# microsoft/GenerativeImage2Text

Hardware: AMD Instinct MI355X
Metric: captions/sec whole-node (GIT_BASE 224px bs=64/GPU greedy len=20) (higher is better)
Workload: dtype f16; 1 GPU; GIT_BASE 224px bs=64/GPU greedy max_len=20 frames=1; global_batch=64, parallelism=dp1, decode_steps_per_caption=19, seq_len_returned=20, hip_graph=True, contexts_in_flight=4, layernorm_folded=True, library=libgitmi_f16.so, encoder_chains=2, schedule=mixed

## Files before the change

generativeimage2text_amd/csrc/kernels_gemm10.hip:

```cpp
#include "gitmi_common.h"
#include "launchers.h"
#include <type_traits>

namespace gitmi {

namespace {

constexpr int BN = 256, BK = 64;
constexpr int HALF_BYTES = 128 * BK * 2;
constexpr int BUF_BYTES = 4 * HALF_BYTES;
constexpr int LDS_BYTES = 2 * BUF_BYTES;
constexpr int SLOT_A0 = 0, SLOT_A1 = HALF_BYTES, SLOT_B0 = 2 * HALF_BYTES, SLOT_B1 = 3 * HALF_BYTES;

typedef __attribute__((address_space(3))) void lds_void_t;

#define P8_BARRIER()                           \
    do {                                       \
        __builtin_amdgcn_sched_barrier(0);     \
        __builtin_amdgcn_s_barrier();          \
        asm volatile("" ::: "memory");         \
        __builtin_amdgcn_sched_barrier(0);     \
    } while (0)

__device__ __forceinline__ float add_unfused(float a, float b) {
#pragma clang fp contract(off)
    return a + b;
}

__device__ __forceinline__ void half_wave_sum2_hi(float& a, float& b) {
    asm volatile(
        "s_nop 1\n\t"
        "v_add_f32_dpp %0, %0, %0 quad_perm:[1,0,3,2] row_mask:0xf bank_mask:0xf\n\t"
        "v_add_f32_dpp %1, %1, %1 quad_perm:[1,0,3,2] row_mask:0xf bank_mask:0xf\n\t"
        "s_nop 0\n\t"
        "v_add_f32_dpp %0, %0, %0 quad_perm:[2,3,0,1] row_mask:0xf bank_mask:0xf\n\t"
        "v_add_f32_dpp %1, %1, %1 quad_perm:[2,3,0,1] row_mask:0xf bank_mask:0xf\n\t"
        "s_nop 0\n\t"
        "v_add_f32_dpp %0, %0, %0 row_ror:4 row_mask:0xf bank_mask:0xf\n\t"
        "v_add_f32_dpp %1, %1, %1 row_ror:4 row_mask:0xf bank_mask:0xf\n\t"
        "s_nop 0\n\t"
        "v_add_f32_dpp %0, %0, %0 row_ror:8 row_mask:0xf bank_mask:0xf\n\t"
        "v_add_f32_dpp %1, %1, %1 row_ror:8 row_mask:0xf bank_mask:0xf\n\t"
        "s_nop 0\n\t"
        "v_add_f32_dpp %0, %0, %0 row_bcast:15 row_mask:0xa bank_mask:0xf\n\t"
        "v_add_f32_dpp %1, %1, %1 row_bcast:15 row_mask:0xa bank_mask:0xf\n\t"
        "s_nop 1"
        : "+v"(a), "+v"(b));
}

#define P8_LDS_BARRIER()                                   \
    do {                                                   \
        asm volatile("s_waitcnt lgkmcnt(0)" ::: "memory"); \
        __builtin_amdgcn_s_barrier();                      \
        asm volatile("" ::: "memory");                     \
    } while (0)

template <typename T> __device__ __forceinline__ uint32_t pack2o(float lo, float hi) {
    if constexpr (std::is_same<T, f16_t>::value) return pack2h(lo, hi);
    else return pack2bf(lo, hi);
}
template <typename T> __device__ __forceinline__ void unpack2o(uint32_t u, float& lo, float& hi) {
    if constexpr (std::is_same<T, f16_t>::value) unpack2h(u, lo, hi);
    else unpack2op(u, lo, hi);
}

template <int N> __device__ __forceinline__ void wait_vm() {
    if constexpr (N == 8) asm volatile("s_waitcnt vmcnt(8)" ::: "memory");
    else if constexpr (N == 4) asm volatile("s_waitcnt vmcnt(4)" ::: "memory");
    else if constexpr (N == 2) asm volatile("s_waitcnt vmcnt(2)" ::: "memory");
    else if constexpr (N == 0) asm volatile("s_waitcnt vmcnt(0)" ::: "memory");
}

template <typename TOut, int ACT, int DBG = 0, int MH = 128, int EPI = 1, int MH1 = MH, int LNF = 0>
__global__ __launch_bounds__(512) void gemm_p8_kernel(GemmArgs g) {
    static_assert(LNF == 0 || sizeof(TOut) == 2, "LayerNorm folding: 16-bit outputs only");
    static_assert(MH % 32 == 0 && MH1 % 32 == 0 && MH1 <= MH && MH <= 128, "half tiles: multiples of 32 rows, second <= first");
    constexpr int BM = MH + MH1, MI = MH / 32, MI1 = MH1 / 32;
    __shared__ __attribute__((aligned(16))) unsigned char smem[LDS_BYTES];

    const int tid = threadIdx.x;
    const int lane = tid & 63;
    const int wave = __builtin_amdgcn_readfirstlane(tid >> 6);
    const int grp = wave >> 2, wc = wave & 3;
    const int l15 = lane & 15, lg = lane >> 4;
    uint64_t ts[8];
    auto stamp = [&](int i) {
        if constexpr ((DBG & 16) != 0) {
            __builtin_amdgcn_sched_barrier(0);
            ts[2 * i] = __builtin_amdgcn_s_memtime();
            ts[2 * i + 1] = __builtin_amdgcn_s_memrealtime();
            __builtin_amdgcn_sched_barrier(0);
        }
    };
    auto stamps_out = [&]() {
        if constexpr ((DBG & 16) != 0) {
            if (tid == 0) {
                uint64_t* o = reinterpret_cast<uint64_t*>(const_cast<float*>(g.res)) + (size_t)blockIdx.x * 8;
#pragma unroll
                for (int i = 0; i < 8; ++i) o[i] = ts[i];
            }
        }
    };
    stamp(0);

    int tile_m, tile_n;
    {
        const int x = blockIdx.x & 7, idx = blockIdx.x >> 3;
        const int ng = g.ng, mg = 8 / ng;
        const int gn = x % ng, gm = x / ng;
        const int tiles_m = (g.M + BM - 1) / BM;
        const int n_lo = gn * g.tiles_n / ng, n_hi = (gn + 1) * g.tiles_n / ng;
        const int nn = n_hi - n_lo;
        const int tg = tiles_m * nn;
        const int lo_t = gm * tg / mg, hi_t = (gm + 1) * tg / mg;
        if (idx >= hi_t - lo_t) return;
        const int L = lo_t + idx;
        tile_m = L / nn;
        tile_n = n_lo + L % nn;
    }
    const int m0 = tile_m * BM, n0 = tile_n * BN;

    const char* __restrict__ Ab = reinterpret_cast<const char*>(g.A);
    const char* __restrict__ Wb = reinterpret_cast<const char*>(g.W);

    const int Rl = lane >> 4, hi = (lane >> 3) & 1, lo = lane & 7;
    uint32_t a_off[2][2], w_off[2][2];
#pragma unroll
    for (int h = 0; h < 2; ++h)
#pragma unroll
        for (int q = 0; q < 2; ++q) {
            const int rr = h * MH + (wave * 2 + q) * 8 + 2 * Rl + (hi ^ q);
            const int ch = lo ^ (q * 4 + Rl);
            int m = m0 + rr;
            m = m < g.M ? m : g.M - 1;
            a_off[h][q] = ((uint32_t)m * (uint32_t)g.lda + ch * 8) * 2u;
            const int rn = h * 128 + (wave * 2 + q) * 8 + 2 * Rl + (hi ^ q);
            w_off[h][q] = ((uint32_t)(n0 + rn) * (uint32_t)g.K + ch * 8) * 2u;
        }
    auto issue = [&](int isw, int half, int kt) {
        if constexpr (DBG & 8) return;
        const char* src = (isw ? Wb : Ab) + (size_t)kt * (BK * 2);
        unsigned char* dst = smem + (kt & 1) * BUF_BYTES + (isw ? SLOT_B0 : SLOT_A0) + half * HALF_BYTES + wave * 2048;
        const uint32_t o0 = isw ? w_off[half][0] : a_off[half][0];
        const uint32_t o1 = isw ? w_off[half][1] : a_off[half][1];
        __builtin_amdgcn_global_load_lds((const void*)(src + o0), (lds_void_t*)(dst), 16, 0, 0);
        __builtin_amdgcn_global_load_lds((const void*)(src + o1), (lds_void_t*)(dst + 1024), 16, 0, 0);
    };

    const int rowpart = (l15 >> 1) * 256 + ((l15 & 1) ^ ((l15 >> 3) & 1)) * 128;
    const int x7 = (l15 >> 1) & 7;
    const int ch0 = ((0 * 4 + lg) ^ x7) * 16;
    const int ch1 = ((1 * 4 + lg) ^ x7) * 16;
    const int a_rd = grp * (MH / 2) * 128 + rowpart;
    const int a_rd1 = grp * (MH1 / 2) * 128 + rowpart + HALF_BYTES;
    const int w_rd = SLOT_B0 + wc * 32 * 128 + rowpart;

    f32x4_t acc[2][2][2][MI];

    bf16x8_t af[MI][2], wf0[2][2], wf1[2][2];

    auto read_a = [&](const unsigned char* sb, auto half_c) {
        if constexpr (DBG & 4) return;
        constexpr int half = decltype(half_c)::value;
        const int base = half ? a_rd1 : a_rd;
#pragma unroll
        for (int i = 0; i < (half ? MI1 : MI); ++i) {
            af[i][0] = *reinterpret_cast<const bf16x8_t*>(sb + base + i * 2048 + ch0);
            af[i][1] = *reinterpret_cast<const bf16x8_t*>(sb + base + i * 2048 + ch1);
        }
    };
    constexpr std::integral_constant<int, 0> H0{};
    constexpr std::integral_constant<int, 1> H1{};
    auto read_w = [&](const unsigned char* sb, int half, bf16x8_t (&wf)[2][2]) {
        if constexpr (DBG & 4) return;
#pragma unroll
        for (int j = 0; j < 2; ++j) {
            wf[j][0] = *reinterpret_cast<const bf16x8_t*>(sb + w_rd + half * HALF_BYTES + j * 2048 + ch0);
            wf[j][1] = *reinterpret_cast<const bf16x8_t*>(sb + w_rd + half * HALF_BYTES + j * 2048 + ch1);
        }
    };
    auto mma = [&](f32x4_t (&c)[2][MI], const bf16x8_t (&wf)[2][2], auto half_c) {
        if constexpr (DBG & 4) return;
        constexpr int MIq = decltype(half_c)::value ? MI1 : MI;
        __builtin_amdgcn_s_setprio(1);
#pragma unroll
        for (int kk = 0; kk < 2; ++kk)
#pragma unroll
            for (int j = 0; j < 2; ++j)
#pragma unroll
                for (int i = 0; i < MIq; ++i)
                    c[j][i] = mfma16(wf[j][kk], af[i][kk], c[j][i]);
        __builtin_amdgcn_s_setprio(0);
    };

    auto ktile = [&](auto mode_c, int t) {
        constexpr int MODE = decltype(mode_c)::value;
        const unsigned char* sb = smem + (t & 1) * BUF_BYTES;
        read_w(sb, 0, wf0);
        __builtin_amdgcn_sched_barrier(0);
        read_a(sb, H0);
        if constexpr (MODE <= 1) { issue(1, 1, t + 1); wait_vm<8>(); } else { wait_vm<2>(); }
        P8_BARRIER();
        mma(acc[0][0], wf0, H0);
        P8_BARRIER();
        read_w(sb, 1, wf1);
        if constexpr (MODE <= 1) { issue(0, 1, t + 1); wait_vm<8>(); } else { wait_vm<0>(); }
        P8_BARRIER();
        mma(acc[0][1], wf1, H0);
        P8_BARRIER();
        read_a(sb, H1);
        if constexpr (MODE == 0) { issue(0, 0, t + 2); wait_vm<8>(); }
        P8_BARRIER();
        mma(acc[1][1], wf1, H1);
        P8_BARRIER();
        if constexpr (MODE == 0) { issue(1, 0, t + 2); wait_vm<8>(); }
        else if constexpr (MODE == 1) { wait_vm<4>(); }
        P8_BARRIER();
        mma(acc[1][0], wf0, H1);
        P8_BARRIER();
    };

    float lmean[2][MI], lrstd[2][MI];
    unsigned char* const ln_lds = smem + BUF_BYTES + SLOT_A1;
    if constexpr (LNF == 1) {
        const int r = lane >> 1, qm = r >> 4, l = r & 15;
        const int MHq = qm ? MH1 : MH, MIq = qm ? MI1 : MI;
        const int ii = wc < MIq ? wc : MIq - 1;
        const int m = m0 + qm * MH + grp * (MHq / 2) + ii * 16 + l;
        const int mc = m < g.M ? m : g.M - 1;
        const char* src = reinterpret_cast<const char*>(g.ln_part) + (size_t)mc * 32 + (lane & 1) * 16;
        __builtin_amdgcn_global_load_lds((const void*)src, (lds_void_t*)(ln_lds + wave * 1024), 16, 0, 0);
    }
    auto ln_rows = [&]() {
        if constexpr (LNF == 1) {
#pragma unroll
            for (int qm = 0; qm < 2; ++qm) {
                const int MIq = qm ? MI1 : MI;
                const int ii = lg < MIq ? lg : MIq - 1;
                const unsigned char* pr = ln_lds + (grp * 4 + ii) * 1024 + (qm * 16 + l15) * 32;
                const f32x4_t p0 = *reinterpret_cast<const f32x4_t*>(pr);
                const f32x4_t p1 = *reinterpret_cast<const f32x4_t*>(pr + 16);
                const float sx = (p0[0] + p0[2]) + (p1[0] + p1[2]);
                const float sq = (p0[1] + p0[3]) + (p1[1] + p1[3]);
                const float mean = sx * g.ln_inv_d;
                const float rstd = rsqrtf(fmaxf(sq * g.ln_inv_d - mean * mean, 0.f) + g.ln_eps);
#pragma unroll
                for (int i = 0; i < MIq; ++i) {
                    lmean[qm][i] = __shfl(mean, i * 16 + l15, 64);
                    lrstd[qm][i] = __shfl(rstd, i * 16 + l15, 64);
                    asm volatile("" : "+v"(lmean[qm][i]), "+v"(lrstd[qm][i]));
                }
            }
            __builtin_amdgcn_sched_barrier(0);
        }
    };
    const int nk = g.K / BK;
    issue(0, 0, 0); issue(1, 0, 0); issue(1, 1, 0); issue(0, 1, 0); issue(0, 0, 1); issue(1, 0, 1);
    wait_vm<8>();
    P8_BARRIER();
    ln_rows();
#pragma unroll
    for (int a = 0; a < 2; ++a)
#pragma unroll
        for (int b = 0; b < 2; ++b)
#pragma unroll
            for (int j = 0; j < 2; ++j)
#pragma unroll
                for (int i = 0; i < MI; ++i) acc[a][b][j][i] = f32x4_t{0.f, 0.f, 0.f, 0.f};
    if (grp == 1) P8_BARRIER();
    stamp(1);
    for (int t = 0; t < nk - 2; ++t) ktile(std::integral_constant<int, 0>{}, t);
    ktile(std::integral_constant<int, 1>{}, nk - 2);
    ktile(std::integral_constant<int, 2>{}, nk - 1);
    if (grp == 0) P8_BARRIER();
    stamp(2);

    constexpr int NQN = sizeof(TOut) == 2 ? 2 : 1;
    constexpr int WCOL = 128 * NQN;
    constexpr int EPC = 16 / (int)sizeof(TOut);
    constexpr int EPS = WCOL + EPC;
    constexpr int CPR = WCOL / EPC;
    static_assert(MH * EPS * sizeof(TOut) <= LDS_BYTES && (MH * CPR) % 512 == 0 && (MH1 * CPR) % 512 == 0, "epilogue slab does not fit");
    TOut* ep = reinterpret_cast<TOut*>(smem);
    TOut* __restrict__ C = reinterpret_cast<TOut*>(g.C);

    if constexpr (DBG & 2) {
        float sum = 0.f;
#pragma unroll
        for (int a = 0; a < 2; ++a)
#pragma unroll
            for (int b = 0; b < 2; ++b)
#pragma unroll
                for (int j = 0; j < 2; ++j)
#pragma unroll
                    for (int i = 0; i < MI; ++i) sum += acc[a][b][j][i][0] + acc[a][b][j][i][1] + acc[a][b][j][i][2] + acc[a][b][j][i][3];
        if (sum == 12345.678f) C[0] = (TOut)0;
        stamp(3);
        stamps_out();
        return;
    }
    f32x4_t bias4[2][2];
#pragma unroll
    for (int qn = 0; qn < 2; ++qn)
#pragma unroll
        for (int j = 0; j < 2; ++j)
            bias4[qn][j] = g.bias ? *reinterpret_cast<const f32x4_t*>(g.bias + n0 + qn * 128 + wc * 32 + j * 16 + lg * 4)
                                  : f32x4_t{0.f, 0.f, 0.f, 0.f};

    f32x4_t cs4[2][2];
    if constexpr (LNF == 1) {
#pragma unroll
        for (int qn = 0; qn < 2; ++qn)
#pragma unroll
            for (int j = 0; j < 2; ++j)
                cs4[qn][j] = *reinterpret_cast<const f32x4_t*>(g.ln_colsum + n0 + qn * 128 + wc * 32 + j * 16 + lg * 4);
    }
    auto ln_apply = [&](float a, int qm, int qn, int j, int i, int r) -> float {
        if constexpr (LNF == 1) return lrstd[qm][i] * fmaf(-lmean[qm][i], cs4[qn][j][r], a);
        else return a;
    };

    if constexpr (sizeof(TOut) == 4 && EPI == 1) {
        float* Cf = reinterpret_cast<float*>(g.C);
        const float* R = g.res;
        const int col0 = n0 + wc * 32 + lg * 4;
        const bool has_res = R != nullptr && !(DBG & 1);
#pragma unroll
        for (int qm = 0; qm < 2; ++qm) {
            const int MIq = qm ? MI1 : MI, MHq = qm ? MH1 : MH;
            f32x4_t rr[MI][2][2];
            if (has_res) {
#pragma unroll
                for (int i = 0; i < MIq; ++i) {
                    const int m = m0 + qm * MH + grp * (MHq / 2) + i * 16 + l15;
                    const int mc = m < g.M ? m : g.M - 1;
                    const float* rp = R + (size_t)mc * g.ldr + col0;
#pragma unroll
                    for (int qn = 0; qn < 2; ++qn)
#pragma unroll
                        for (int j = 0; j < 2; ++j)
                            rr[i][qn][j] = *reinterpret_cast<const f32x4_t*>(rp + qn * 128 + j * 16);
                }
            }
#pragma unroll
            for (int i = 0; i < MIq; ++i) {
                const int m = m0 + qm * MH + grp * (MHq / 2) + i * 16 + l15;
                float* cp = Cf + (size_t)m * g.ldc + col0;
                const bool ok = m < g.M && !(DBG & 1);
#pragma unroll
                for (int qn = 0; qn < 2; ++qn)
#pragma unroll
                    for (int j = 0; j < 2; ++j) {
                        f32x4_t v;
#pragma unroll
                        for (int r = 0; r < 4; ++r) v[r] = apply_act_t<ACT>(acc[qm][qn][j][i][r] + bias4[qn][j][r]);
                        if (has_res) {
#pragma unroll
                            for (int r = 0; r < 4; ++r) v[r] = add_unfused(v[r], rr[i][qn][j][r]);
                        }
                        if (ok) *reinterpret_cast<f32x4_t*>(cp + qn * 128 + j * 16) = v;
                    }
            }
        }
        return;
    }

    float rgm[8], rbt[8];
    if constexpr (LNF == 2) {
        if (g.res_part) {
            ld8(g.res_gamma + n0 + (tid & 31) * 8, rgm);
            ld8(g.res_beta + n0 + (tid & 31) * 8, rbt);
        }
    }
#pragma unroll
    for (int qm = 0; qm < 2; ++qm)
#pragma unroll
        for (int s = 0; s < 2 / NQN; ++s) {
            const int MIq = qm ? MI1 : MI, MHq = qm ? MH1 : MH;
#pragma unroll
            for (int u = 0; u < NQN; ++u) {
                const int qn = s * NQN + u;
#pragma unroll
                for (int j = 0; j < 2; ++j) {
                    const int nl = u * 128 + wc * 32 + j * 16 + lg * 4;
#pragma unroll
                    for (int i = 0; i < MIq; ++i) {
                        float v[4];
#pragma unroll
                        for (int r = 0; r < 4; ++r) v[r] = apply_act_t<ACT>(ln_apply(acc[qm][qn][j][i][r], qm, qn, j, i, r) + bias4[qn][j][r]);
                        TOut* p = ep + (grp * (MHq / 2) + i * 16 + l15) * EPS + nl;
                        if constexpr (sizeof(TOut) == 4) {
                            *reinterpret_cast<f32x4_t*>(p) = f32x4_t{v[0], v[1], v[2], v[3]};
                        } else {
                            uint2 t2;
                            t2.x = pack2o<TOut>(v[0], v[1]);
                            t2.y = pack2o<TOut>(v[2], v[3]);
                            *reinterpret_cast<uint2*>(p) = t2;
                        }
                    }
                }
            }
            P8_LDS_BARRIER();
#pragma unroll 4
            for (int q = 0; q < MHq * CPR / 512; ++q) {
                const int chunk = tid + q * 512;
                const int row = chunk / CPR, cc = chunk % CPR;
                const int m = m0 + qm * MH + row;
                const int n = n0 + s * WCOL + cc * EPC;
                if (m < g.M && !(DBG & 1)) {
                    if constexpr (sizeof(TOut) == 4) {
                        f32x4_t v = *reinterpret_cast<const f32x4_t*>(ep + row * EPS + cc * EPC);
                        if (g.res && !(DBG & 16)) {
                            const f32x4_t rr = *reinterpret_cast<const f32x4_t*>(g.res + (size_t)m * g.ldr + n);
                            v[0] += rr[0]; v[1] += rr[1]; v[2] += rr[2]; v[3] += rr[3];
                        }
                        *reinterpret_cast<f32x4_t*>(C + (size_t)m * g.ldc + n) = v;
                    } else if constexpr (LNF == 2) {
                    } else {
                        u32x4_t v = *reinterpret_cast<const u32x4_t*>(ep + row * EPS + cc * EPC);
                        if (g.res && !(DBG & 16)) {
                            float f[8], rs[8];
#pragma unroll
                            for (int e = 0; e < 4; ++e) unpack2o<TOut>(v[e], f[2 * e], f[2 * e + 1]);
                            if constexpr (std::is_same<TOut, f16_t>::value) {
                                const u32x4_t rr = *reinterpret_cast<const u32x4_t*>(reinterpret_cast<const f16_t*>(g.res) + (size_t)m * g.ldr + n);
#pragma unroll
                                for (int e = 0; e < 4; ++e) unpack2h(rr[e], rs[2 * e], rs[2 * e + 1]);
                            } else {
                                const float* rp = g.res + (size_t)m * g.ldr + n;
                                const f32x4_t r0 = *reinterpret_cast<const f32x4_t*>(rp);
                                const f32x4_t r1 = *reinterpret_cast<const f32x4_t*>(rp + 4);
#pragma unroll
                                for (int e = 0; e < 4; ++e) { rs[e] = r0[e]; rs[4 + e] = r1[e]; }
                            }
#pragma unroll
                            for (int e = 0; e < 8; ++e) f[e] += rs[e];
#pragma unroll
                            for (int e = 0; e < 4; ++e) v[e] = pack2o<TOut>(f[2 * e], f[2 * e + 1]);
                        }
                        TOut* cp = C + (size_t)m * g.ldc + n;
                        if (g.dbg & 512)
                            *reinterpret_cast<u32x4_t*>(cp) = v;
                        else
                            asm volatile("global_store_dwordx4 %0, %1, off sc1\n\ts_nop 1" ::"v"(cp), "v"(v) : "memory");
                    }
                }
                if constexpr (LNF == 2) {
                    static_assert(LNF != 2 || CPR == 32, "one stream row per half wave");
                    const bool ok = m < g.M;
                    const int mc = ok ? m : g.M - 1;
                    u32x4_t v = *reinterpret_cast<const u32x4_t*>(ep + row * EPS + cc * EPC);
                    float f[8];
#pragma unroll
                    for (int e = 0; e < 4; ++e) unpack2h(v[e], f[2 * e], f[2 * e + 1]);
                    if (g.res) {
                        float rs[8];
                        const u32x4_t rr = *reinterpret_cast<const u32x4_t*>(reinterpret_cast<const f16_t*>(g.res) + (size_t)mc * g.ldr + n);
#pragma unroll
                        for (int e = 0; e < 4; ++e) unpack2h(rr[e], rs[2 * e], rs[2 * e + 1]);
                        if (g.res_part) {
                            const f32x4_t* pp = reinterpret_cast<const f32x4_t*>(g.res_part + (size_t)mc * 4);
                            const f32x4_t p0 = pp[0], p1 = pp[1];
                            const float mean = ((p0[0] + p0[2]) + (p1[0] + p1[2])) * g.res_inv_d;
                            const float rstd = rsqrtf(fmaxf(((p0[1] + p0[3]) + (p1[1] + p1[3])) * g.res_inv_d - mean * mean, 0.f) + g.res_eps);
#pragma unroll
                            for (int e = 0; e < 8; ++e) rs[e] = fmaf((rs[e] - mean) * rstd, rgm[e], rbt[e]);
                        }
#pragma unroll
                        for (int e = 0; e < 8; ++e) f[e] += rs[e];
#pragma unroll
                        for (int e = 0; e < 4; ++e) v[e] = pack2h(f[2 * e], f[2 * e + 1]);
                    }
                    if (g.part_out) {
                        typedef __attribute__((ext_vector_type(2))) float f32x2_t;
                        f32x2_t s2 = {0.f, 0.f}, q2 = {0.f, 0.f};
#pragma unroll
                        for (int e = 0; e < 4; ++e) {
                            float x0, x1;
                            unpack2h(v[e], x0, x1);
                            const f32x2_t x = {x0, x1};
                            s2 += x;
                            q2 = __builtin_elementwise_fma(x, x, q2);
                        }
                        float sx = s2[0] + s2[1], sq = q2[0] + q2[1];
                        half_wave_sum2_hi(sx, sq);
                        if (ok && cc == 16 && !(DBG & 1)) g.part_out[(size_t)m * 4 + tile_n] = float2{sx, sq};
                    }
                    if (ok && !(DBG & 1)) {
                        TOut* cp = C + (size_t)m * g.ldc + n;
                        asm volatile("global_store_dwordx4 %0, %1, off sc1\n\ts_nop 1" ::"v"(cp), "v"(v) : "memory");
                    }
                }
            }
            P8_LDS_BARRIER();
        }
    if constexpr ((DBG & 16) != 0) {
        asm volatile("s_waitcnt vmcnt(0)" ::: "memory");
        stamp(3);
        stamps_out();
    }
}

}

template <typename TOut, int MH, int EPI = 1, int MH1 = MH, int LNF = 0>
static void launch_p8_t(const GemmArgs& g, hipStream_t s) {
    if constexpr (LNF == 2) {
        hipLaunchKernelGGL((gemm_p8_kernel<TOut, GITMI_ACT_NONE, 0, MH, EPI, MH1, LNF>), dim3(g.nwg), dim3(512), 0, s, g);
        return;
    } else {
    if (g.dbg && LNF == 0) {
        if constexpr (MH == 128 && MH1 == 128) {
            switch (g.dbg) {
                case 1: hipLaunchKernelGGL((gemm_p8_kernel<TOut, 0, 1>), dim3(g.nwg), dim3(512), 0, s, g); return;
                case 2: hipLaunchKernelGGL((gemm_p8_kernel<TOut, 0, 2>), dim3(g.nwg), dim3(512), 0, s, g); return;
                case 6: hipLaunchKernelGGL((gemm_p8_kernel<TOut, 0, 6>), dim3(g.nwg), dim3(512), 0, s, g); return;
                case 10: hipLaunchKernelGGL((gemm_p8_kernel<TOut, 0, 10>), dim3(g.nwg), dim3(512), 0, s, g); return;
#ifdef GITMI_PROBE
                case 16: hipLaunchKernelGGL((gemm_p8_kernel<TOut, 0, 16>), dim3(g.nwg), dim3(512), 0, s, g); return;
                case 17: hipLaunchKernelGGL((gemm_p8_kernel<TOut, 0, 17>), dim3(g.nwg), dim3(512), 0, s, g); return;
                case 18: hipLaunchKernelGGL((gemm_p8_kernel<TOut, 0, 18>), dim3(g.nwg), dim3(512), 0, s, g); return;
                case 22: hipLaunchKernelGGL((gemm_p8_kernel<TOut, 0, 22>), dim3(g.nwg), dim3(512), 0, s, g); return;
                case 26: hipLaunchKernelGGL((gemm_p8_kernel<TOut, 0, 26>), dim3(g.nwg), dim3(512), 0, s, g); return;
#endif
                default: break;
            }
        }
    }
    switch (g.act) {
        case GITMI_ACT_QUICKGELU:
            hipLaunchKernelGGL((gemm_p8_kernel<TOut, GITMI_ACT_QUICKGELU, 0, MH, EPI, MH1, LNF>), dim3(g.nwg), dim3(512), 0, s, g); break;
        case GITMI_ACT_GELU_ERF:
            hipLaunchKernelGGL((gemm_p8_kernel<TOut, GITMI_ACT_GELU_ERF, 0, MH, EPI, MH1, LNF>), dim3(g.nwg), dim3(512), 0, s, g); break;
        default:
            hipLaunchKernelGGL((gemm_p8_kernel<TOut, GITMI_ACT_NONE, 0, MH, EPI, MH1, LNF>), dim3(g.nwg), dim3(512), 0, s, g); break;
    }
    }
}

bool gemm_p8_supports(const GemmArgs& g) {
    return g.K % BK == 0 && g.K >= 2 * BK && g.N % BN == 0 &&
           (double)g.M * g.lda * 2.0 < 4.0e9 && (double)g.N * g.K * 2.0 < 4.0e9;
}

static int p8_xcd_count(const GemmArgs& g, int bm, int ng, int* max_nn_out) {
    const int tiles_m = (g.M + bm - 1) / bm, tiles_n = g.N / BN, mg = 8 / ng;
    int max_cnt = 0, max_nn = 0;
    for (int x = 0; x < 8; ++x) {
        const int gn = x % ng, gm = x / ng;
        const int nn = (gn + 1) * tiles_n / ng - gn * tiles_n / ng;
        const int tg = tiles_m * nn;
        const int cnt = (gm + 1) * tg / mg - gm * tg / mg;
        max_cnt = cnt > max_cnt ? cnt : max_cnt;
        max_nn = nn > max_nn ? nn : max_nn;
    }
    if (max_nn_out) *max_nn_out = max_nn;
    return max_cnt;
}
static int p8_plan(const GemmArgs& g, int bm, int* ng_out, int* max_cnt_out) {
    const int tiles_n = g.N / BN;
    int best_ng = 1, best_rounds = 1 << 30, best_cnt = 0, best_panels = 1 << 30;
    for (int ng = 1; ng <= 8 && ng <= tiles_n; ng *= 2) {
        int max_nn = 0;
        const int max_cnt = p8_xcd_count(g, bm, ng, &max_nn);
        const int rounds = (max_cnt + 31) / 32;
        const int panels = (32 + max_nn - 1) / max_nn + (max_nn < 32 ? max_nn : 32);
        if (rounds < best_rounds || (rounds == best_rounds && panels < best_panels)) {
            best_ng = ng; best_rounds = rounds; best_cnt = max_cnt; best_panels = panels;
        }
    }
    if (ng_out) *ng_out = best_ng;
    if (max_cnt_out) *max_cnt_out = best_cnt;
    return best_rounds;
}

int gemm_p8_cost(const GemmArgs& g, int bm) {
    const int rounds = p8_plan(g, bm, nullptr, nullptr);
    const int ktile = 1450 * (90 + 166 * bm / 256) / 256;
    return rounds * (1450 + (g.K / BK) * ktile + 4700 * bm / 256);
}

template <int MH, int MH1>
static void launch_p8_height(const GemmArgs& g, bool out_f32, bool staged, hipStream_t s) {
#ifdef GITMI_OPS_F16
    if (g.ln_part) { launch_p8_t<bf16_t, MH, 1, MH1, 1>(g, s); return; }
    if (g.part_out || g.res_part) { launch_p8_t<f16_t, MH, 1, MH1, 2>(g, s); return; }
#endif
    if (g.out_f16) launch_p8_t<f16_t, MH, 1, MH1>(g, s);
    else if (!out_f32) launch_p8_t<bf16_t, MH, 1, MH1>(g, s);
    else if (staged) launch_p8_t<float, MH, 0, MH1>(g, s);
    else launch_p8_t<float, MH, 1, MH1>(g, s);
}

hipError_t launch_gemm_p8(GemmArgs g, bool out_f32, hipStream_t s) {
    if (g.ln_part || g.part_out || g.res_part) {
#ifndef GITMI_OPS_F16
        return hipErrorInvalidValue;
#endif
        if (g.ln_part && (out_f32 || g.out_f16 || g.res || !g.ln_colsum || g.ln_nparts < 1 || g.part_out || g.res_part)) return hipErrorInvalidValue;
        if ((g.part_out || g.res_part) && (!g.out_f16 || out_f32 || g.act != 0 || g.N > 1024)) return hipErrorInvalidValue;
        if (g.res_part && (!g.res || !g.res_gamma || !g.res_beta || g.res_nparts < 1)) return hipErrorInvalidValue;
    }
    static const int heights[5] = {256, 224, 192, 160, 128};
    int bm = 256;
    if (!g.shared) {
        int best = gemm_p8_cost(g, 256);
        for (int h = 1; h < 5; ++h) {
            const int c = gemm_p8_cost(g, heights[h]);
            if (c < best) { best = c; bm = heights[h]; }
        }
    }
    if (g.dbg & 64) bm = 192;
    if (g.dbg & 128) bm = 256;
    if (g.dbg & 16384) bm = 160;
    if (g.dbg & 32768) bm = 224;
    if (g.dbg & 65536) bm = 128;
    g.dbg &= ~(64 | 128 | 16384 | 32768 | 65536);
    g.tiles_n = g.N / BN;
    int max_cnt = 0;
    p8_plan(g, bm, &g.ng, &max_cnt);
    if (g.dbg & (1024 | 2048 | 4096 | 8192)) {
        const int ng = (g.dbg & 1024) ? 1 : (g.dbg & 2048) ? 2 : (g.dbg & 4096) ? 4 : 8;
        g.dbg &= ~(1024 | 2048 | 4096 | 8192);
        if (ng <= g.tiles_n) { g.ng = ng; max_cnt = p8_xcd_count(g, bm, ng, nullptr); }
    }
    g.nwg = 8 * max_cnt;
    const bool staged = (g.dbg & 256) != 0;
    g.dbg &= ~256;
    switch (bm) {
        case 224: launch_p8_height<128, 96>(g, out_f32, staged, s); break;
        case 192: launch_p8_height<96, 96>(g, out_f32, staged, s); break;
        case 160: launch_p8_height<96, 64>(g, out_f32, staged, s); break;
        case 128: launch_p8_height<64, 64>(g, out_f32, staged, s); break;
        default: launch_p8_height<128, 128>(g, out_f32, staged, s); break;
    }
    return hipGetLastError();
}

}
```

Baseline: 11510 captions/s.

## Park LayerNorm row stats in LDS and pack epilogue math into float2

Per-row LayerNorm mean and rstd are no longer held in registers through the main loop. They are written to an extra LDS region and reloaded only in the epilogue, which is meant to cut VGPR pressure during the MMA loop. The bias, LN fold and activation math is rewritten on float2 vectors so it can use packed FP32 instructions. Store addressing is hoisted into a per-thread slab pointer, and the residual add is skipped for LNF paths. This adds LDS usage and a dependence on the layout of the parked stats.

```diff
diff --git a/generativeimage2text_amd/csrc/kernels_gemm10.hip b/generativeimage2text_amd/csrc/kernels_gemm10.hip
--- a/generativeimage2text_amd/csrc/kernels_gemm10.hip
+++ b/generativeimage2text_amd/csrc/kernels_gemm10.hip
@@ -64,6 +64,34 @@
     else unpack2op(u, lo, hi);
 }
 
+typedef __attribute__((ext_vector_type(2))) float f32x2_t;
+template <int ACT> __device__ __forceinline__ f32x2_t apply_act2(f32x2_t x) {
+    if constexpr (ACT == GITMI_ACT_QUICKGELU) {
+        const f32x2_t a = (x * -1.702f) * 1.4426950408889634f;
+        const f32x2_t d = f32x2_t{__builtin_amdgcn_exp2f(a[0]), __builtin_amdgcn_exp2f(a[1])} + 1.0f;
+        return x * f32x2_t{fast_rcp(d[0]), fast_rcp(d[1])};
+    } else if constexpr (ACT == GITMI_ACT_GELU_ERF) {
+        const f32x2_t one = {1.0f, 1.0f};
+        const f32x2_t z = x * 0.70710678118654752440f;
+        const f32x2_t az = __builtin_elementwise_abs(z);
+        const f32x2_t d = __builtin_elementwise_fma(f32x2_t{0.3275911f, 0.3275911f}, az, one);
+        const f32x2_t t = {fast_rcp(d[0]), fast_rcp(d[1])};
+        f32x2_t poly = {1.061405429f, 1.061405429f};
+        poly = __builtin_elementwise_fma(poly, t, f32x2_t{-1.453152027f, -1.453152027f});
+        poly = __builtin_elementwise_fma(poly, t, f32x2_t{1.421413741f, 1.421413741f});
+        poly = __builtin_elementwise_fma(poly, t, f32x2_t{-0.284496736f, -0.284496736f});
+        poly = __builtin_elementwise_fma(poly, t, f32x2_t{0.254829592f, 0.254829592f});
+        poly = poly * t;
+        const f32x2_t a = (-az * az) * 1.4426950408889634f;
+        const f32x2_t ex = {__builtin_amdgcn_exp2f(a[0]), __builtin_amdgcn_exp2f(a[1])};
+        const f32x2_t e = __builtin_elementwise_fma(-poly, ex, one);
+        const f32x2_t se = {copysignf(e[0], z[0]), copysignf(e[1], z[1])};
+        return (x * 0.5f) * (se + 1.0f);
+    } else {
+        return x;
+    }
+}
+
 template <int N> __device__ __forceinline__ void wait_vm() {
     if constexpr (N == 8) asm volatile("s_waitcnt vmcnt(8)" ::: "memory");
     else if constexpr (N == 4) asm volatile("s_waitcnt vmcnt(4)" ::: "memory");
@@ -76,7 +104,8 @@
     static_assert(LNF == 0 || sizeof(TOut) == 2, "LayerNorm folding: 16-bit outputs only");
     static_assert(MH % 32 == 0 && MH1 % 32 == 0 && MH1 <= MH && MH <= 128, "half tiles: multiples of 32 rows, second <= first");
     constexpr int BM = MH + MH1, MI = MH / 32, MI1 = MH1 / 32;
-    __shared__ __attribute__((aligned(16))) unsigned char smem[LDS_BYTES];
+    constexpr int PARK_BYTES = LNF == 1 ? 8 * 2 * 16 * 4 * (int)sizeof(float2) : 0;
+    __shared__ __attribute__((aligned(16))) unsigned char smem[LDS_BYTES + PARK_BYTES];
 
     const int tid = threadIdx.x;
     const int lane = tid & 63;
@@ -220,7 +249,7 @@
         P8_BARRIER();
     };
 
-    float lmean[2][MI], lrstd[2][MI];
+    float2* const ln_park = reinterpret_cast<float2*>(smem + LDS_BYTES);
     unsigned char* const ln_lds = smem + BUF_BYTES + SLOT_A1;
     if constexpr (LNF == 1) {
         const int r = lane >> 1, qm = r >> 4, l = r & 15;
@@ -244,12 +273,7 @@
                 const float sq = (p0[1] + p0[3]) + (p1[1] + p1[3]);
                 const float mean = sx * g.ln_inv_d;
                 const float rstd = rsqrtf(fmaxf(sq * g.ln_inv_d - mean * mean, 0.f) + g.ln_eps);
-#pragma unroll
-                for (int i = 0; i < MIq; ++i) {
-                    lmean[qm][i] = __shfl(mean, i * 16 + l15, 64);
-                    lrstd[qm][i] = __shfl(rstd, i * 16 + l15, 64);
-                    asm volatile("" : "+v"(lmean[qm][i]), "+v"(lrstd[qm][i]));
-                }
+                ln_park[((wave * 2 + qm) * 16 + l15) * 4 + lg] = float2{mean, rstd};
             }
             __builtin_amdgcn_sched_barrier(0);
         }
@@ -315,10 +339,6 @@
             for (int j = 0; j < 2; ++j)
                 cs4[qn][j] = *reinterpret_cast<const f32x4_t*>(g.ln_colsum + n0 + qn * 128 + wc * 32 + j * 16 + lg * 4);
     }
-    auto ln_apply = [&](float a, int qm, int qn, int j, int i, int r) -> float {
-        if constexpr (LNF == 1) return lrstd[qm][i] * fmaf(-lmean[qm][i], cs4[qn][j][r], a);
-        else return a;
-    };
 
     if constexpr (sizeof(TOut) == 4 && EPI == 1) {
         float* Cf = reinterpret_cast<float*>(g.C);
@@ -377,6 +397,16 @@
 #pragma unroll
         for (int s = 0; s < 2 / NQN; ++s) {
             const int MIq = qm ? MI1 : MI, MHq = qm ? MH1 : MH;
+            f32x2_t lmr[MI];
+            if constexpr (LNF == 1) {
+                const f32x4_t* pk = reinterpret_cast<const f32x4_t*>(ln_park + ((wave * 2 + qm) * 16 + l15) * 4);
+#pragma unroll
+                for (int h = 0; h < (MIq + 1) / 2; ++h) {
+                    const f32x4_t v4 = pk[h];
+                    lmr[2 * h] = f32x2_t{v4[0], v4[1]};
+                    if (2 * h + 1 < MIq) lmr[2 * h + 1] = f32x2_t{v4[2], v4[3]};
+                }
+            }
 #pragma unroll
             for (int u = 0; u < NQN; ++u) {
                 const int qn = s * NQN + u;
@@ -387,7 +417,20 @@
                     for (int i = 0; i < MIq; ++i) {
                         float v[4];
 #pragma unroll
-                        for (int r = 0; r < 4; ++r) v[r] = apply_act_t<ACT>(ln_apply(acc[qm][qn][j][i][r], qm, qn, j, i, r) + bias4[qn][j][r]);
+                        for (int h = 0; h < 2; ++h) {
+                            f32x2_t x = {acc[qm][qn][j][i][2 * h], acc[qm][qn][j][i][2 * h + 1]};
+                            const f32x2_t b2 = {bias4[qn][j][2 * h], bias4[qn][j][2 * h + 1]};
+                            if constexpr (LNF == 1) {
+                                const f32x2_t c2 = {cs4[qn][j][2 * h], cs4[qn][j][2 * h + 1]};
+                                const f32x2_t mean2 = {lmr[i][0], lmr[i][0]}, rstd2 = {lmr[i][1], lmr[i][1]};
+                                x = __builtin_elementwise_fma(rstd2, __builtin_elementwise_fma(-mean2, c2, x), b2);
+                            } else {
+                                x = x + b2;
+                            }
+                            x = apply_act2<ACT>(x);
+                            v[2 * h] = x[0];
+                            v[2 * h + 1] = x[1];
+                        }
                         TOut* p = ep + (grp * (MHq / 2) + i * 16 + l15) * EPS + nl;
                         if constexpr (sizeof(TOut) == 4) {
                             *reinterpret_cast<f32x4_t*>(p) = f32x4_t{v[0], v[1], v[2], v[3]};
@@ -401,12 +444,14 @@
                 }
             }
             P8_LDS_BARRIER();
+            constexpr int RPQ = 512 / CPR;
+            const int cc = tid % CPR;
+            const int n = n0 + s * WCOL + cc * EPC;
+            TOut* const cslab = C + (size_t)(m0 + qm * MH + tid / CPR) * g.ldc + n;
 #pragma unroll 4
             for (int q = 0; q < MHq * CPR / 512; ++q) {
-                const int chunk = tid + q * 512;
-                const int row = chunk / CPR, cc = chunk % CPR;
+                const int row = tid / CPR + q * RPQ;
                 const int m = m0 + qm * MH + row;
-                const int n = n0 + s * WCOL + cc * EPC;
                 if (m < g.M && !(DBG & 1)) {
                     if constexpr (sizeof(TOut) == 4) {
                         f32x4_t v = *reinterpret_cast<const f32x4_t*>(ep + row * EPS + cc * EPC);
@@ -418,7 +463,7 @@
                     } else if constexpr (LNF == 2) {
                     } else {
                         u32x4_t v = *reinterpret_cast<const u32x4_t*>(ep + row * EPS + cc * EPC);
-                        if (g.res && !(DBG & 16)) {
+                        if (LNF == 0 && g.res && !(DBG & 16)) {
                             float f[8], rs[8];
 #pragma unroll
                             for (int e = 0; e < 4; ++e) unpack2o<TOut>(v[e], f[2 * e], f[2 * e + 1]);
@@ -438,7 +483,7 @@
 #pragma unroll
                             for (int e = 0; e < 4; ++e) v[e] = pack2o<TOut>(f[2 * e], f[2 * e + 1]);
                         }
-                        TOut* cp = C + (size_t)m * g.ldc + n;
+                        TOut* cp = cslab + (size_t)(q * RPQ) * g.ldc;
                         if (g.dbg & 512)
                             *reinterpret_cast<u32x4_t*>(cp) = v;
                         else
```

Measured after the change: 11540 captions/s, median of 5. No clear change (+0.2%).
